# hruffieux/atlasqtl

Measured on NVIDIA B200. Metric: SNPxtrait CAVI updates/s, higher is better.
Workload: dtype f64

## Files before the change

### atlasqtl_b200/csrc/aq_sweep.cuh

```cuda
#pragma once
#include "aq_common.cuh"
#include "aq_mis.cuh"
#ifdef AQ_TIMING
#define AQ_T(i) do { long long t_ = clock64(); tacc[i] += t_ - tlast; tlast = t_; } while (0)
#define AQ_T0() long long tlast = clock64()
#else
#define AQ_T(i) do { } while (0)
#define AQ_T0() do { } while (0)
#endif

#ifndef AQ_S_FINISH_AT
#define AQ_S_FINISH_AT -1
#endif

namespace aq {

struct SweepParams {
    const int* order;
    const double* xtiles;
    size_t tile_stride;
    int nb;
    int ntiles;
    int k_base;
    int q;
    int q_pad;
    int ld_resid;
    int ncta;
    double* resid;
    double* gam;
    double* mu;
    const double* dtab;
    const double* wtab;
    const double* i0tab;
    const double* tau;
    const double* log_tau;
    const double* sig2_beta;
    double c;
    double log_sig2_inv;
    double* cs_gam;
    double* cs_gmu2;
    double* cs_b2;
    double* rsq;
    double* cs_z;
    double* rowpart;
    int rowpart_base;
    int p_pad;
    int mode;
    int nseg;
    int seg_len;
    int* seg_done;
    const unsigned long long* mbits;
    int mwords;
    const double* xnsq;
    const double* atab;
    const double* ltab;
    const double* gk;
    double* mis_out;
    long long* timing;
};

constexpr int kMaxCluster = 8;

template <int MT_, int NT_, bool CL_ = false, bool MIS_ = false>
struct SweepCfg {
    static constexpr bool kMis = MIS_;
    static constexpr int WS = 14;
    static constexpr int MT = MT_;
    static constexpr int NT = NT_;
    static constexpr bool kCl = CL_;
    static constexpr int kMmaWarps = WS;
    static constexpr int kT = MT * 8;
    static constexpr int kNPad = WS * NT * 8;
    static constexpr int kXS = kNPad + ((kNPad % 16 == 0) ? 8 : 0);
    static constexpr int kThreads = 16 * 32;
    static constexpr int kStages = 3;
    static constexpr bool kShortLogistic = CL_ || MIS_ || MT_ != 2;
    static constexpr int kSFin = (MT_ <= 2) ? AQ_S_FINISH_AT : -1;
    static constexpr size_t kTileDoubles = (size_t)kBlk * kXS + kTileTail;
    static constexpr int kSps = 8;
    static constexpr size_t kSpartDoubles = (size_t)WS * kT * kSps;
    static constexpr bool kChainSums = MT > 1;
    static constexpr bool kHelperSumsFollowers = kCl && kChainSums;
#ifdef AQ_AB_CHAIN_FWD
    static constexpr bool kChainForwards = kCl && kChainSums;
#else
    static constexpr bool kChainForwards = false;
#endif
    static constexpr size_t kSsumDoubles = (kChainSums && !kHelperSumsFollowers) ? 0 : (size_t)2 * kT * kSps;
    static constexpr size_t kDbufDoubles = (size_t)2 * kT * kBlk;
    static constexpr size_t kRsqDoubles = (size_t)WS * kT;
    static constexpr int kIoPer = kMis ? 4 : 2;
    static constexpr size_t kIoDoubles = (size_t)2 * kBlk * kIoPer * kT;
    static constexpr int kStgArrays = kMis ? 8 : 5;
    static constexpr size_t kStgDoubles = (size_t)kStgArrays * kBlk * kT;
    static constexpr size_t kGkDoubles = kMis ? (size_t)2 * 128 * kT : 0;
    static constexpr uint32_t kDeltaBytes = (uint32_t)(kT * kBlk * sizeof(double));
    static constexpr size_t kRedDoubles = kCl ? (size_t)2 * (kMaxCluster - 1) * kT * kSps : 0;
    static constexpr size_t kRsqAllDoubles = kCl ? (size_t)(kMaxCluster - 1) * kT : 0;
    static constexpr int kNumBars = 2 * kStages + 2 + 2 + 2 + 1 + 2 + 1 + 8;
    static constexpr size_t kSmemBytes = (kStages * kTileDoubles + kSpartDoubles + kSsumDoubles + kDbufDoubles + kRsqDoubles +
                                          kIoDoubles + kStgDoubles + kRedDoubles + kRsqAllDoubles + kGkDoubles) *
                                             sizeof(double) +
                                         24 * sizeof(uint64_t);
    static_assert(kNumBars <= 24, "barrier block");
    static_assert(kT <= 32, "one chain lane per trait");
    static_assert(!kMis || kT == 16, "the missing-response variant uses 16-trait tiles (its Gram band table is laid out for them)");
    static_assert(kXS % 16 == 8, "row stride must be 8 mod 16 doubles");
    static_assert(kSmemBytes <= 232448, "shared memory budget (227 KB)");
};

__device__ __forceinline__ int sp_off(int r, int t) { return r * 8 + ((((t >> 1) ^ (r >> 1)) & 3) << 1) + (t & 1); }
template <int kT>
__device__ __forceinline__ int d_off(int r, int t) { return (t >> 1) * 2 * kT + ((2 * r + (t & 1)) ^ (((t >> 1) & 1) << 3)); }

template <int N>
__device__ __forceinline__ void group_sums(double (&v)[N], int lane, int top_bit) {
    if constexpr (N > 1) {
        const bool up = (lane & top_bit) != 0;
        double w[N / 2];
#pragma unroll
        for (int i = 0; i < N / 2; ++i) {
            const double send = up ? v[i] : v[i + N / 2];
            const double keep = up ? v[i + N / 2] : v[i];
            w[i] = keep + __shfl_xor_sync(0xffffffffu, send, top_bit);
        }
        group_sums<N / 2>(w, lane, top_bit >> 1);
        v[0] = w[0];
    } else {
        v[0] += __shfl_xor_sync(0xffffffffu, v[0], 2);
        v[0] += __shfl_xor_sync(0xffffffffu, v[0], 1);
    }
}

template <class Cfg>
__device__ __forceinline__ void sum_own_partials(double (&s)[kBlk], const double* spart, uint64_t* sdone, uint64_t* sfree,
                                                 long gb, int lane, int tsum) {
    constexpr int WS = Cfg::WS, kT = Cfg::kT;
    static_assert(WS == 14, "MMA warp i sits on SMSP i % 3 for i < 12, warps 12 and 13 on SMSP 3");
    constexpr int kH = (kT <= 16) ? 2 : 1;
    const int half = (kH == 2) ? (lane >> 4) : 0;
    const uint32_t par = (uint32_t)((gb >> 1) & 1);
#pragma unroll
    for (int t = 0; t < kBlk; ++t) s[t] = 0.0;
    auto add = [&](int w) {
#pragma unroll
        for (int t = 0; t < kBlk; t += 2) {
            const double2 v = *reinterpret_cast<const double2*>(spart + w * kT * Cfg::kSps + sp_off(tsum, t));
            s[t] += v.x;
            s[t + 1] += v.y;
        }
    };
    mbar_wait(&sdone[(gb & 1) * 4 + 3], par);
    if (kH == 2) add(12 + half);
    else { add(12); add(13); }
#pragma unroll
    for (int g4 = 0; g4 < 3; ++g4) {
        mbar_wait(&sdone[(gb & 1) * 4 + g4], par);
        if (kH == 2) { add(g4 + 6 * half); add(g4 + 6 * half + 3); }
        else { add(g4); add(g4 + 3); add(g4 + 6); add(g4 + 9); }
    }
    __syncwarp();
    if (lane == 0) mbar_arrive(&sfree[0]);
}

template <class Cfg>
__device__ __forceinline__ void sum_follower_tiles(double (&s)[kBlk], const double* red, uint64_t* sred, long gb, int ncta,
                                                   int lane, int tsum) {
    constexpr int kT = Cfg::kT;
    constexpr int kH = (kT <= 16) ? 2 : 1;
    const int half = (kH == 2) ? (lane >> 4) : 0;
#pragma unroll
    for (int t = 0; t < kBlk; ++t) s[t] = 0.0;
    if (lane == 0) mbar_arrive_expect_tx(&sred[gb & 1], (uint32_t)(ncta - 1) * Cfg::kDeltaBytes);
    mbar_wait(&sred[gb & 1], (uint32_t)((gb >> 1) & 1));
    const int mid = (kH == 2) ? (ncta + 1) / 2 : ncta;
    for (int r2 = (half == 0 ? 1 : mid); r2 < (half == 0 ? mid : ncta); ++r2) {
        const double* rp = red + (size_t)((gb & 1) * (kMaxCluster - 1) + (r2 - 1)) * kT * Cfg::kSps;
#pragma unroll
        for (int t = 0; t < kBlk; t += 2) {
            const double2 v = *reinterpret_cast<const double2*>(rp + sp_off(tsum, t));
            s[t] += v.x;
            s[t + 1] += v.y;
        }
    }
    if (kH == 2) {
#pragma unroll
        for (int t = 0; t < kBlk; ++t) s[t] += __shfl_xor_sync(0xffffffffu, s[t], 16);
    }
}

template <class Cfg>
__device__ __forceinline__ void sum_s_partials(double (&s)[kBlk], const double* spart, const double* red, uint64_t* sdone,
                                               uint64_t* sfree, uint64_t* sred, long gb, int ncta, int lane, int tsum) {
    constexpr int kT = Cfg::kT;
    constexpr int kH = (kT <= 16) ? 2 : 1;
    const int half = (kH == 2) ? (lane >> 4) : 0;
    sum_own_partials<Cfg>(s, spart, sdone, sfree, gb, lane, tsum);
    if (Cfg::kCl && ncta > 1) {
        if (lane == 0) mbar_arrive_expect_tx(&sred[gb & 1], (uint32_t)(ncta - 1) * Cfg::kDeltaBytes);
        mbar_wait(&sred[gb & 1], (uint32_t)((gb >> 1) & 1));
        if (half == 0) {
            for (int r2 = 1; r2 < ncta; ++r2) {
                const double* rp = red + (size_t)((gb & 1) * (kMaxCluster - 1) + (r2 - 1)) * kT * Cfg::kSps;
#pragma unroll
                for (int t = 0; t < kBlk; t += 2) {
                    const double2 v = *reinterpret_cast<const double2*>(rp + sp_off(tsum, t));
                    s[t] += v.x;
                    s[t + 1] += v.y;
                }
            }
        }
    }
    if (kH == 2) {
#pragma unroll
        for (int t = 0; t < kBlk; ++t) s[t] += __shfl_xor_sync(0xffffffffu, s[t], 16);
    }
}

struct Unit {
    int tile, seg, b0, b1;
};
__device__ __forceinline__ Unit unit_of(const SweepParams& P, int group, int ngroups, int ju) {
    const int u = group + ju * ngroups;
    Unit w;
    w.seg = u / P.ntiles;
    w.tile = u - w.seg * P.ntiles;
    w.b0 = w.seg * P.seg_len;
    w.b1 = min(P.nb, w.b0 + P.seg_len);
    return w;
}
__device__ __forceinline__ void unit_acquire(const SweepParams& P, const Unit& w, int lane) {
    if (w.seg > 0) {
        if (lane == 0) {
            uint32_t spins = 0;
            while (ld_acquire_gpu(P.seg_done + w.tile) < w.seg) {
                __nanosleep(64);
                if (++spins == (1u << 23)) __trap();
            }
        }
        __syncwarp();
    }
}
template <class Cfg>
__device__ __forceinline__ void unit_release(const SweepParams& P, const Unit& w) {
    if (P.nseg > 1) {
        __syncwarp();
        if constexpr (Cfg::kCl) cluster_sync_all();
        else asm volatile("bar.sync 2, %0;" ::"n"(Cfg::kThreads) : "memory");
        bool leader = threadIdx.x == 0;
        if constexpr (Cfg::kCl) leader = leader && cluster_ctarank() == 0;
        if (leader) {
            __threadfence();
            st_release_gpu(P.seg_done + w.tile, w.seg + 1);
        }
    }
}

template <class Cfg>
__global__ void __launch_bounds__(Cfg::kThreads, 1) sweep_kernel(const SweepParams P) {
    constexpr int WS = Cfg::WS, MT = Cfg::MT, NT = Cfg::NT, kT = Cfg::kT, XS = Cfg::kXS;
    constexpr int kStages = Cfg::kStages;
    constexpr bool kCl = Cfg::kCl;
    constexpr bool kMis = Cfg::kMis;
    constexpr int kIoPer = Cfg::kIoPer;
    extern __shared__ __align__(128) unsigned char smem_raw[];
    double* tiles = reinterpret_cast<double*>(smem_raw);
    double* spart = tiles + kStages * Cfg::kTileDoubles;
    double* ssum = spart + Cfg::kSpartDoubles;
    double* dbuf = ssum + Cfg::kSsumDoubles;
    double* rsqs = dbuf + Cfg::kDbufDoubles;
    double* iobuf = rsqs + Cfg::kRsqDoubles;
    double* stg = iobuf + Cfg::kIoDoubles;
    double* red = stg + Cfg::kStgDoubles;
    double* rsq_all = red + Cfg::kRedDoubles;
    double* gkbuf = rsq_all + Cfg::kRsqAllDoubles;
    uint64_t* bars = reinterpret_cast<uint64_t*>(gkbuf + Cfg::kGkDoubles);
    uint64_t* full = bars;
    uint64_t* empty = bars + kStages;
    uint64_t* dready = bars + 2 * kStages;
    uint64_t* dcons = bars + 2 * kStages + 2;
    uint64_t* sred = bars + 2 * kStages + 4;
    uint64_t* rsqbar = bars + 2 * kStages + 6;
    uint64_t* inready = bars + 2 * kStages + 7;
    uint64_t* sfree = bars + 2 * kStages + 9;
    uint64_t* sdone = bars + 2 * kStages + 10;

    const int wid = threadIdx.x >> 5, lane = threadIdx.x & 31;
#ifdef AQ_TIMING
    long long tacc[16] = {0, 0, 0, 0, 0, 0, 0, 0, 0, 0, 0, 0, 0, 0, 0, 0};
#endif
    const int smsp = wid & 3, quad = wid >> 2;
    const bool is_mma = smsp != 3 || quad >= 2;
    const int mma_idx = smsp != 3 ? quad * 3 + smsp : 12 + (quad - 2);
    const bool is_chain = smsp == 3 && quad == 0;
    const bool is_helper = smsp == 3 && quad == 1;
    const bool is_producer = mma_idx == Cfg::kMmaWarps - 1 && is_mma;
    const int ncta = kCl ? P.ncta : 1;
    const int rank = kCl ? (int)cluster_ctarank() : 0;
    const int group = kCl ? (int)cluster_id_x() : (int)blockIdx.x;
    const int ngroups = kCl ? (int)cluster_count_x() : (int)gridDim.x;
    if (threadIdx.x == 0) {
        for (int s = 0; s < kStages; ++s) { mbar_init(&full[s], 1); mbar_init(&empty[s], Cfg::kMmaWarps); }
        for (int s = 0; s < 2; ++s) {
            for (int g4 = 0; g4 < 4; ++g4) mbar_init(&sdone[s * 4 + g4], g4 < 3 ? 4 : Cfg::kMmaWarps - 12);
            mbar_init(&dready[s], 1);
            mbar_init(&dcons[s], Cfg::kMmaWarps * ncta);
            mbar_init(&sred[s], 1);
            mbar_init(&inready[s], 1);
        }
        mbar_init(&rsqbar[0], ncta > 1 ? ncta - 1 : 1);
        mbar_init(&sfree[0], 1);
        fence_mbar_init();
    }
    __syncthreads();
    if (kCl) cluster_sync_all();

    const int nunits = P.ntiles * P.nseg;
    const int my_units = (nunits - group + ngroups - 1) / ngroups;
    const uint32_t tile_bytes = (uint32_t)(Cfg::kTileDoubles * sizeof(double));

    if (is_mma) {
        const int ws = mma_idx;
        const int mtid = mma_idx * 32 + lane;
        long total = 0;
        int pj = 0, pb = 0, pb1 = 0;
        if (is_producer) {
            for (int ju = 0; ju < my_units; ++ju) {
                const Unit w = unit_of(P, group, ngroups, ju);
                total += w.b1 - w.b0;
            }
            if (my_units > 0) {
                const Unit w = unit_of(P, group, ngroups, 0);
                pb = w.b0;
                pb1 = w.b1;
            }
        }
        auto load_next = [&](long it) {
            const int stage = (int)(it % kStages);
            mbar_arrive_expect_tx(&full[stage], tile_bytes);
            bulk_g2s(tiles + stage * Cfg::kTileDoubles, P.xtiles + ((size_t)pb * ncta + rank) * P.tile_stride, tile_bytes, &full[stage]);
            if (++pb == pb1 && ++pj < my_units) {
                const Unit w = unit_of(P, group, ngroups, pj);
                pb = w.b0;
                pb1 = w.b1;
            }
        };
        if (is_producer && lane == 0)
            for (long it = 0; it < kStages && it < total; ++it) load_next(it);
        const int g = lane >> 2, l = lane & 3;
        const int i0 = ws * NT * 8;
        const int ig = rank * Cfg::kNPad + i0;
        constexpr int tr0 = 0;
        const int offS = g * XS + ((i0 + 2 * l) ^ ((g & 2) << 1));
        const int offU0 = l * XS + ((i0 + g) ^ ((l & 2) << 1));
        const int offU1 = (l + 4) * XS + ((i0 + g) ^ ((l & 2) << 1));
        const int offD = d_off<kT>(tr0 + g, l);
        const int offP = sp_off(tr0 + g, 2 * l);
        uint32_t dcons_leader[2] = {0, 0}, rsqbar_leader = 0, rsq_all_leader = 0;
        if (kCl) {
            dcons_leader[0] = mapa_u32(&dcons[0], 0);
            dcons_leader[1] = mapa_u32(&dcons[1], 0);
            rsqbar_leader = mapa_u32(&rsqbar[0], 0);
            rsq_all_leader = mapa_u32(rsq_all, 0);
        }
        double acc[MT][NT][2];
        long gb = 0;
        for (int ju = 0; ju < my_units; ++ju) {
            const Unit un = unit_of(P, group, ngroups, ju);
            const int k0 = P.k_base + un.tile * kT;
            unit_acquire(P, un, lane);
#pragma unroll
            for (int mt = 0; mt < MT; ++mt)
#pragma unroll
                for (int nt = 0; nt < NT; ++nt) {
                    const double2 v = __ldcg(reinterpret_cast<const double2*>(
                        P.resid + (size_t)(k0 + tr0 + mt * 8 + g) * P.ld_resid + ig + nt * 8 + 2 * l));
                    acc[mt][nt][0] = v.x;
                    acc[mt][nt][1] = v.y;
                }
            constexpr int kSC = (MT >= 4) ? 1 : 2;
            double sa[MT][2][2];
            uint32_t mb[MT];
            if constexpr (kMis) {
#pragma unroll
                for (int mt = 0; mt < MT; ++mt) {
                    const unsigned long long* row = P.mbits + (size_t)(k0 + tr0 + mt * 8 + g) * P.mwords;
                    uint32_t bits = 0;
#pragma unroll
                    for (int nt = 0; nt < NT; ++nt)
#pragma unroll
                        for (int e = 0; e < 2; ++e) {
                            const int smp = ig + nt * 8 + 2 * l + e;
                            bits |= (uint32_t)((__ldg(row + (smp >> 6)) >> (smp & 63)) & 1ull) << (2 * nt + e);
                        }
                    mb[mt] = bits;
                }
            }
            auto s_issue = [&](long gbi) {
                const int stage = (int)(gbi % kStages);
                AQ_T0();
                mbar_wait(&full[stage], (uint32_t)((gbi / kStages) & 1));
                AQ_T(10);
                const double* xt = tiles + stage * Cfg::kTileDoubles;
#pragma unroll
                for (int mt = 0; mt < MT; ++mt) sa[mt][0][0] = sa[mt][0][1] = sa[mt][1][0] = sa[mt][1][1] = 0.0;
#pragma unroll
                for (int nt = 0; nt < NT; ++nt) {
                    const double2 xb = *reinterpret_cast<const double2*>(xt + offS + nt * 8);
#pragma unroll
                    for (int mt = 0; mt < MT; ++mt) dmma(sa[mt][0][0], sa[mt][0][1], acc[mt][nt][0], xb.x);
#pragma unroll
                    for (int mt = 0; mt < MT; ++mt) dmma(sa[mt][kSC - 1][0], sa[mt][kSC - 1][1], acc[mt][nt][1], xb.y);
                }
                AQ_T(11);
            };
            auto s_finish = [&](long gbi) {
                AQ_T0();
                if (gbi > 0) mbar_wait(&sfree[0], (uint32_t)((gbi - 1) & 1));
                AQ_T(12);
                double* sp = spart + (size_t)ws * kT * Cfg::kSps + offP;
#pragma unroll
                for (int mt = 0; mt < MT; ++mt) {
                    double2 v;
                    v.x = (kSC == 2) ? sa[mt][0][0] + sa[mt][1][0] : sa[mt][0][0];
                    v.y = (kSC == 2) ? sa[mt][0][1] + sa[mt][1][1] : sa[mt][0][1];
                    *reinterpret_cast<double2*>(sp + mt * 8 * Cfg::kSps) = v;
                }
                __syncwarp();
                if (lane == 0) mbar_arrive(&sdone[(gbi & 1) * 4 + smsp]);
                AQ_T(13);
            };
            if (P.mode == 0) {
                s_issue(gb);
                s_finish(gb);
            }
            for (int b = un.b0; b < un.b1; ++b, ++gb) {
                const bool s_next = P.mode == 0 && b + 1 < un.b1;
                if (s_next) s_issue(gb + 1);
                if (Cfg::kSFin < 0 && s_next) s_finish(gb + 1);
                const int stage = (int)(gb % kStages);
                AQ_T0();
                if (P.mode != 0) mbar_wait(&full[stage], (uint32_t)((gb / kStages) & 1));
                mbar_wait(&dready[gb & 1], (uint32_t)((gb >> 1) & 1));
                AQ_T(14);
                const double* xt = tiles + stage * Cfg::kTileDoubles;
                const double* db = dbuf + (size_t)(gb & 1) * kT * kBlk;
                if (kCl && rank == 0 && !(Cfg::kChainForwards && P.mode == 0)) {
                    constexpr int kV2 = kT * kBlk / 2;
                    const int nsend = (ncta - 1) * kV2;
                    for (int L = mtid; L < nsend; L += Cfg::kMmaWarps * 32) {
                        const int r2 = 1 + L / kV2, idx = L % kV2;
                        const double2 v = *reinterpret_cast<const double2*>(db + 2 * idx);
                        st_async_v2(mapa_u32(db + 2 * idx, r2), v.x, v.y, mapa_u32(&dready[gb & 1], r2));
                    }
                }
                double nd[MT][2];
#pragma unroll
                for (int mt = 0; mt < MT; ++mt) {
                    nd[mt][0] = db[offD + 16 * mt];
                    nd[mt][1] = db[offD + 16 * mt + 4 * kT];
                }
                if (P.mode != 0) {
                    __syncwarp();
                    if (lane == 0) {
                        if (kCl) mbar_arrive_cluster(dcons_leader[gb & 1]);
                        else mbar_arrive(&dcons[gb & 1]);
                    }
                }
#pragma unroll
                for (int nt = 0; nt < NT; nt += 2) {
                    constexpr int kLast = NT - 1;
                    const int nt1 = nt + 1 < NT ? nt + 1 : kLast;
                    const bool two = nt + 1 < NT;
                    const double x0a = xt[offU0 + nt * 8], x1a = xt[offU1 + nt * 8];
                    const double x0b = xt[offU0 + nt1 * 8], x1b = xt[offU1 + nt1 * 8];
#pragma unroll
                    for (int mt = 0; mt < MT; ++mt) dmma(acc[mt][nt][0], acc[mt][nt][1], nd[mt][0], x0a);
                    if (two) {
#pragma unroll
                        for (int mt = 0; mt < MT; ++mt) dmma(acc[mt][nt1][0], acc[mt][nt1][1], nd[mt][0], x0b);
                    }
#pragma unroll
                    for (int mt = 0; mt < MT; ++mt) dmma(acc[mt][nt][0], acc[mt][nt][1], nd[mt][1], x1a);
                    if (two) {
#pragma unroll
                        for (int mt = 0; mt < MT; ++mt) dmma(acc[mt][nt1][0], acc[mt][nt1][1], nd[mt][1], x1b);
                    }
                    if (nt == Cfg::kSFin && s_next) s_finish(gb + 1);
                }
                if (Cfg::kSFin >= NT && s_next) s_finish(gb + 1);
                if constexpr (kMis) {
#pragma unroll
                    for (int mt = 0; mt < MT; ++mt)
#pragma unroll
                        for (int nt = 0; nt < NT; ++nt) {
                            if (!((mb[mt] >> (2 * nt)) & 1u)) acc[mt][nt][0] = 0.0;
                            if (!((mb[mt] >> (2 * nt + 1)) & 1u)) acc[mt][nt][1] = 0.0;
                        }
                }
                __syncwarp();
                if (lane == 0) mbar_arrive(&empty[stage]);
                AQ_T(15);
                if (is_producer) {
                    if (lane == 0 && gb + kStages < total) {
                        mbar_wait(&empty[stage], (uint32_t)((gb / kStages) & 1));
                        load_next(gb + kStages);
                    }
                    __syncwarp();
                }
            }
#pragma unroll
            for (int mt = 0; mt < MT; ++mt) {
                double ss = 0.0;
#pragma unroll
                for (int nt = 0; nt < NT; ++nt) {
                    double2 v;
                    v.x = acc[mt][nt][0];
                    v.y = acc[mt][nt][1];
                    ss = fma(v.x, v.x, ss);
                    ss = fma(v.y, v.y, ss);
                    *reinterpret_cast<double2*>(P.resid + (size_t)(k0 + tr0 + mt * 8 + g) * P.ld_resid + ig + nt * 8 + 2 * l) = v;
                }
                ss += __shfl_xor_sync(0xffffffffu, ss, 1);
                ss += __shfl_xor_sync(0xffffffffu, ss, 2);
                if (l == 0) rsqs[ws * kT + tr0 + mt * 8 + g] = ss;
            }
            const bool last_seg = un.seg == P.nseg - 1;
            asm volatile("bar.sync 1, %0;" ::"n"(Cfg::kMmaWarps * 32) : "memory");
            if (mtid < 32 * ((kT + 31) / 32)) {
                double ss = 0.0;
                if (mtid < kT) {
#pragma unroll
                    for (int w2 = 0; w2 < WS; ++w2) ss += rsqs[w2 * kT + mtid];
                }
                if (!kCl) {
                    if (last_seg && mtid < kT && k0 + mtid < P.q) P.rsq[k0 + mtid] = ss;
                } else if (rank != 0) {
                    if (mtid < kT) st_cluster_f64(rsq_all_leader + (uint32_t)(((rank - 1) * kT + mtid) * sizeof(double)), ss);
                    __syncwarp();
                    if (mtid == 0) mbar_arrive_cluster(rsqbar_leader);
                } else {
                    if (ncta > 1) mbar_wait_cluster(&rsqbar[0], (uint32_t)(ju & 1));
                    if (mtid < kT) {
                        for (int r2 = 1; r2 < ncta; ++r2) ss += rsq_all[(r2 - 1) * kT + mtid];
                        if (last_seg && k0 + mtid < P.q) P.rsq[k0 + mtid] = ss;
                    }
                }
            }
            asm volatile("bar.sync 1, %0;" ::"n"(Cfg::kMmaWarps * 32) : "memory");
            unit_release<Cfg>(P, un);
        }
    } else if (is_chain && rank != 0) {
        constexpr int kH = (kT <= 16) ? 2 : 1;
        constexpr int kTP = kBlk / kH;
        const int half = (kH == 2) ? (lane >> 4) : 0;
        const int tl = (kH == 2) ? (lane & 15) : lane;
        const bool active = tl < kT;
        const int tls = active ? tl : 0;
        const uint32_t red_leader = mapa_u32(red, 0);
        const uint32_t sred_leader[2] = {mapa_u32(&sred[0], 0), mapa_u32(&sred[1], 0)};
        long gb = 0;
        for (int ju = 0; ju < my_units; ++ju) {
            const Unit un = unit_of(P, group, ngroups, ju);
            for (int b = un.b0; b < un.b1; ++b, ++gb) {
                if (gb >= 2) mbar_wait(&dready[gb & 1], (uint32_t)(((gb >> 1) - 1) & 1));
                if (lane == 0) mbar_arrive_expect_tx(&dready[gb & 1], Cfg::kDeltaBytes);
                if (P.mode != 0) continue;
                double s[kBlk];
                sum_own_partials<Cfg>(s, spart, sdone, sfree, gb, lane, tls);
                if (kH == 2) {
#pragma unroll
                    for (int t = 0; t < kBlk; ++t) s[t] += __shfl_xor_sync(0xffffffffu, s[t], 16);
                }
                if (active) {
                    const uint32_t dst = red_leader + (uint32_t)((((gb & 1) * (kMaxCluster - 1)) + (rank - 1)) * kT *
                                                                 Cfg::kSps * sizeof(double));
#pragma unroll
                    for (int i = 0; i < kTP; i += 2) {
                        const int t = half * kTP + i;
                        st_async_v2(dst + (uint32_t)sp_off(tl, t) * (uint32_t)sizeof(double), s[t], s[t + 1], sred_leader[gb & 1]);
                    }
                }
            }
            unit_release<Cfg>(P, un);
        }
    } else if (is_helper) {
        constexpr int kH = (kT <= 16) ? 2 : 1;
        constexpr int kTP = kBlk / kH;
        constexpr bool kStageWI = (kH == 2);
        const int half = (kH == 2) ? (lane >> 4) : 0;
        const int tl = (kH == 2) ? (lane & 15) : lane;
        const bool active = tl < kT;
        const int tls = active ? tl : 0;
        const int t0 = half * kTP;
        const bool work = P.mode == 0 && rank == 0;
        int idn[kTP], idc[kTP];
        double wn[kTP], in[kTP];
        long gb = 0;
        for (int ju = 0; ju < my_units; ++ju) {
            const Unit un = unit_of(P, group, ngroups, ju);
            if (work) {
                const int tile = un.tile;
                const int k = P.k_base + tile * kT + tls;
                const bool valid = active && k < P.q;
                double cst;
                if constexpr (kMis) cst = -(P.log_tau[k] + P.log_sig2_inv) / 2;
                else cst = -(P.log_tau[k] + P.log_sig2_inv + log(P.sig2_beta[k])) / 2;
                const double ctau = P.c * P.tau[k], inv_ctau = 1.0 / ctau;
                double sg = 0.0, sgm2 = 0.0, sb2 = 0.0, sz = 0.0;
                double ss2g = 0.0, sxgm2 = 0.0, sxs2g = 0.0, sxb2 = 0.0, sgl = 0.0;
                double xnn[kTP], s2n[kTP], lsn[kTP];
                double* rowrow = P.rowpart ? P.rowpart + (size_t)(P.rowpart_base + tile) * P.p_pad : nullptr;
                auto stage_rows = [&](int blk) {
                    constexpr int kLanesPerRow = kT / 2, kRowsPerInst = 32 / kLanesPerRow;
                    constexpr int kArrays = kMis ? 8 : (kStageWI ? 5 : 3);
                    static_assert(!kMis || kStageWI, "the missing-response variant stages all its rows");
                    const int idr = __ldg(P.order + (size_t)blk * kBlk + (lane & 7));
                    const int rsub = lane / kLanesPerRow, csub = 2 * (lane % kLanesPerRow);
                    const size_t kcol = (size_t)P.k_base + (size_t)tile * kT + csub;
#pragma unroll
                    for (int r0 = 0; r0 < kArrays * kBlk; r0 += kRowsPerInst) {
                        const int row = r0 + rsub;
                        const int a = row / kBlk, t = row % kBlk;
                        const int idt = __shfl_sync(0xffffffffu, idr, t);
                        if (row < kArrays * kBlk) {
                            const double* base = a == 0 ? P.gam : a == 1 ? P.mu : a == 2 ? P.dtab : a == 3 ? P.wtab :
                                                 a == 4 ? P.i0tab : a == 5 ? P.xnsq : a == 6 ? P.atab : P.ltab;
                            cp_async16(stg + (size_t)row * kT + csub, base + (size_t)(idt < 0 ? 0 : idt) * P.q_pad + kcol);
                        }
                    }
                    cp_async_commit();
                };
                auto stage_gk = [&](long g, int blk) {
                    if constexpr (kMis) {
                        const double* src = P.gk + (((size_t)(P.k_base / kT + tile) * P.nb + blk) * 128) * kT;
                        double* dst = gkbuf + (size_t)(g & 1) * 128 * kT;
                        for (int i = lane; i < 128 * kT / 2; i += 32) cp_async16(dst + 2 * i, src + 2 * i);
                        cp_async_commit();
                    }
                };
                auto pre = [&](long g, int blk) {
                    AQ_T0();
                    double* io = iobuf + (size_t)(g & 1) * kBlk * kIoPer * kT;
                    cp_async_wait_all();
                    __syncwarp();
#pragma unroll
                    for (int i = 0; i < kTP; ++i) {
                        const int t = t0 + i;
                        idn[i] = __ldg(P.order + (size_t)blk * kBlk + t);
                        const double go = stg[(0 * kBlk + t) * kT + tls], mo = stg[(1 * kBlk + t) * kT + tls];
                        const double dd = stg[(2 * kBlk + t) * kT + tls];
                        if (kStageWI) {
                            wn[i] = stg[(3 * kBlk + t) * kT + tls];
                            in[i] = stg[(4 * kBlk + t) * kT + tls];
                        }
                        if constexpr (kMis) {
                            const double xn = stg[(5 * kBlk + t) * kT + tls], aa = stg[(6 * kBlk + t) * kT + tls];
                            const double ls = stg[(7 * kBlk + t) * kT + tls];
                            xnn[i] = xn;
                            s2n[i] = aa * inv_ctau;
                            lsn[i] = ls;
                            if (active) {
                                io[(t * kIoPer + 0) * kT + tl] = idn[i] >= 0 ? go * mo : 0.0;
                                io[(t * kIoPer + 1) * kT + tl] = P.c * (dd - 0.5 * ls + cst);
                                io[(t * kIoPer + 2) * kT + tl] = aa;
                                io[(t * kIoPer + 3) * kT + tl] = 0.5 * P.c * aa * ctau;
                            }
                        } else if (active) {
                            io[(t * kIoPer + 0) * kT + tl] = idn[i] >= 0 ? go * mo : 0.0;
                            io[(t * kIoPer + 1) * kT + tl] = P.c * (dd + cst);
                        }
                    }
                    if (blk + 1 < un.b1) stage_rows(blk + 1);
                    if constexpr (Cfg::kHelperSumsFollowers) {
                        if (ncta > 1) {
                            double s[kBlk];
                            sum_follower_tiles<Cfg>(s, red, sred, g, ncta, lane, tls);
                            if (half == 0 && active) {
#pragma unroll
                                for (int t = 0; t < kBlk; t += 2) {
                                    double2 v;
                                    v.x = s[t];
                                    v.y = s[t + 1];
                                    *reinterpret_cast<double2*>(ssum + (size_t)(g & 1) * kT * Cfg::kSps + sp_off(tl, t)) = v;
                                }
                            }
                        }
                    }
                    if (!Cfg::kChainSums) {
                        AQ_T(4);
                        double s[kBlk];
                        sum_s_partials<Cfg>(s, spart, red, sdone, sfree, sred, g, ncta, lane, tls);
                        if (half == 0 && active) {
#pragma unroll
                            for (int t = 0; t < kBlk; t += 2) {
                                double2 v;
                                v.x = s[t];
                                v.y = s[t + 1];
                                *reinterpret_cast<double2*>(ssum + (size_t)(g & 1) * kT * Cfg::kSps + sp_off(tl, t)) = v;
                            }
                        }
                    }
                    __syncwarp();
                    if (lane == 0) mbar_arrive(&inready[g & 1]);
                    AQ_T(7);
                };
                auto post = [&](long g, int blk, const double (&ww)[kTP], const double (&ii)[kTP], const double (&xc)[kTP],
                                const double (&s2c)[kTP], const double (&lsc)[kTP]) {
                    AQ_T0();
                    mbar_wait(&dready[g & 1], (uint32_t)((g >> 1) & 1));
                    AQ_T(8);
                    if (blk + 2 < un.b1) stage_gk(g + 2, blk + 2);
                    const double* io = iobuf + (size_t)(g & 1) * kBlk * kIoPer * kT;
                    double zrow[kTP];
#pragma unroll
                    for (int i = 0; i < kTP; ++i) {
                        const int t = t0 + i;
                        const double gm = io[(t * kIoPer + 0) * kT + tls];
                        const double m = io[(t * kIoPer + 1) * kT + tls];
                        zrow[i] = 0.0;
                        if (idc[i] >= 0) {
                            const double bn = gm * m;
                            const double z = fma(gm, ww[i], ii[i]);
                            sg += gm;
                            sgm2 = fma(bn, m, sgm2);
                            sb2 = fma(bn, bn, sb2);
                            sz += z;
                            if constexpr (kMis) {
                                ss2g = fma(s2c[i], gm, ss2g);
                                sxgm2 = fma(xc[i] * bn, m, sxgm2);
                                sxs2g = fma(xc[i] * s2c[i], gm, sxs2g);
                                sxb2 = fma(xc[i] * bn, bn, sxb2);
                                sgl = fma(gm, lsc[i], sgl);
                            }
                            if (valid) {
                                const size_t off = (size_t)idc[i] * P.q_pad + k;
                                P.gam[off] = gm;
                                P.mu[off] = m;
                                if (!kCl) zrow[i] = z;
                            }
                        }
                    }
                    if (!kCl && P.rowpart) {
                        group_sums<kTP>(zrow, lane, kH == 2 ? 8 : 16);
                        const int slot = (lane >> 2) & (kTP - 1);
                        int ids = idc[0];
#pragma unroll
                        for (int i = 1; i < kTP; ++i) ids = slot == i ? idc[i] : ids;
                        if ((lane & 3) == 0 && ids >= 0) rowrow[ids] = zrow[0];
                    }
                    AQ_T(9);
                };
                stage_gk(gb, un.b0);
                if (un.b0 + 1 < un.b1) stage_gk(gb + 1, un.b0 + 1);
                stage_rows(un.b0);
                pre(gb, un.b0);
                for (int b = un.b0; b < un.b1; ++b, ++gb) {
                    double ww[kTP], ii[kTP], xc[kTP], s2c[kTP], lsc[kTP];
#pragma unroll
                    for (int i = 0; i < kTP; ++i) {
                        idc[i] = idn[i];
                        xc[i] = xnn[i];
                        s2c[i] = s2n[i];
                        lsc[i] = lsn[i];
                        if (kStageWI) {
                            ww[i] = wn[i];
                            ii[i] = in[i];
                        } else {
                            const size_t off = (size_t)(idc[i] < 0 ? 0 : idc[i]) * P.q_pad + k;
                            ww[i] = P.wtab[off];
                            ii[i] = P.i0tab[off];
                        }
                    }
                    if (b + 1 < un.b1) pre(gb + 1, b + 1);
                    post(gb, b, ww, ii, xc, s2c, lsc);
                }
                if (kH == 2) {
                    sg += __shfl_xor_sync(0xffffffffu, sg, 16);
                    sgm2 += __shfl_xor_sync(0xffffffffu, sgm2, 16);
                    sb2 += __shfl_xor_sync(0xffffffffu, sb2, 16);
                    sz += __shfl_xor_sync(0xffffffffu, sz, 16);
                    if constexpr (kMis) {
                        ss2g += __shfl_xor_sync(0xffffffffu, ss2g, 16);
                        sxgm2 += __shfl_xor_sync(0xffffffffu, sxgm2, 16);
                        sxs2g += __shfl_xor_sync(0xffffffffu, sxs2g, 16);
                        sxb2 += __shfl_xor_sync(0xffffffffu, sxb2, 16);
                        sgl += __shfl_xor_sync(0xffffffffu, sgl, 16);
                    }
                }
                unit_acquire(P, un, lane);
                if constexpr (kMis) {
                    if (valid && half == 0) {
                        double* o = P.mis_out + k;
                        o[(size_t)kMisGam * P.q_pad] = sg;
                        o[(size_t)kMisGamMu2 * P.q_pad] = sgm2;
                        o[(size_t)kMisS2Gam * P.q_pad] = ss2g;
                        o[(size_t)kMisXnGamMu2 * P.q_pad] = sxgm2;
                        o[(size_t)kMisXnS2Gam * P.q_pad] = sxs2g;
                        o[(size_t)kMisXnBeta2 * P.q_pad] = sxb2;
                        o[(size_t)kMisZ * P.q_pad] = sz;
                        o[(size_t)kMisGamLogS2 * P.q_pad] = sgl;
                    }
                } else if (valid && half == 0) {
                    if (un.seg > 0) {
                        sg += __ldcg(P.cs_gam + k);
                        sgm2 += __ldcg(P.cs_gmu2 + k);
                        sb2 += __ldcg(P.cs_b2 + k);
                        sz += __ldcg(P.cs_z + k);
                    }
                    P.cs_gam[k] = sg;
                    P.cs_gmu2[k] = sgm2;
                    P.cs_b2[k] = sb2;
                    P.cs_z[k] = sz;
                }
            }
            unit_release<Cfg>(P, un);
        }
    } else if (is_chain) {
        const int tl = lane;
        const bool active = tl < kT;
        const int tls = active ? tl : 0;
        const int tsum0 = (kT <= 16) ? (lane & 15) : lane;
        const int tsum = tsum0 < kT ? tsum0 : 0;
        auto publish = [&](long gb, const double (&nd)[kBlk]) {
            double* dblk = dbuf + (size_t)(gb & 1) * kT * kBlk;
            if constexpr (Cfg::kChainForwards) {
                if (P.mode == 0 && active) {
                    for (int r2 = 1; r2 < ncta; ++r2) {
                        const uint32_t rbar = mapa_u32(&dready[gb & 1], r2);
#pragma unroll
                        for (int t = 0; t < kBlk; t += 2)
                            st_async_v2(mapa_u32(dblk + d_off<kT>(tl, t), r2), nd[t], nd[t + 1], rbar);
                    }
                }
            }
            if (active) {
#pragma unroll
                for (int t = 0; t < kBlk; t += 2) {
                    double2 v;
                    v.x = nd[t];
                    v.y = nd[t + 1];
                    *reinterpret_cast<double2*>(dblk + d_off<kT>(tl, t)) = v;
                }
            }
            __syncwarp();
            if (lane == 0) mbar_arrive(&dready[gb & 1]);
        };
        long gb = 0;
        for (int ju = 0; ju < my_units; ++ju) {
            const Unit un = unit_of(P, group, ngroups, ju);
            const int k = P.k_base + un.tile * kT + tls;
            const bool valid = active && k < P.q;
            if (P.mode == 0) {
                double a = 0.0, bq = 0.0;
                if constexpr (!kMis) {
                    const double sig2 = P.sig2_beta[k];
                    a = P.c * sig2 * P.tau[k];
                    bq = P.c * a * a / (2.0 * sig2);
                }
                double corr[kBlk];
#pragma unroll
                for (int t = 0; t < kBlk; ++t) corr[t] = 0.0;
                for (int b = un.b0; b < un.b1; ++b, ++gb) {
                    AQ_T0();
                    const int stage = (int)(gb % kStages);
                    mbar_wait(&full[stage], (uint32_t)((gb / kStages) & 1));
                    const double* gband = kMis ? gkbuf + (size_t)(gb & 1) * 128 * kT + tsum
                                               : tiles + stage * Cfg::kTileDoubles + kBlk * XS;
                    constexpr int gstride = kMis ? kT : 1;
                    double* io = iobuf + (size_t)(gb & 1) * kBlk * kIoPer * kT;
                    double s[kBlk], bo[kBlk], ap[kBlk], nd[kBlk], av[kMis ? kBlk : 1], bv[kMis ? kBlk : 1];
                    if constexpr (Cfg::kHelperSumsFollowers) {
                        AQ_T(0);
                        sum_own_partials<Cfg>(s, spart, sdone, sfree, gb, lane, tsum);
                        if (kT <= 16) {
#pragma unroll
                            for (int t = 0; t < kBlk; ++t) s[t] += __shfl_xor_sync(0xffffffffu, s[t], 16);
                        }
                    }
                    mbar_wait(&inready[gb & 1], (uint32_t)((gb >> 1) & 1));
#pragma unroll
                    for (int t = 0; t < kBlk; ++t) {
                        bo[t] = io[(t * kIoPer + 0) * kT + tsum];
                        ap[t] = io[(t * kIoPer + 1) * kT + tsum];
                        if constexpr (kMis) {
                            av[t] = io[(t * kIoPer + 2) * kT + tsum];
                            bv[t] = io[(t * kIoPer + 3) * kT + tsum];
                        }
                    }
                    if constexpr (Cfg::kHelperSumsFollowers) {
                        if (ncta > 1) {
                            const double* sp0 = ssum + (size_t)(gb & 1) * kT * Cfg::kSps;
#pragma unroll
                            for (int t = 0; t < kBlk; t += 2) {
                                const double2 v = *reinterpret_cast<const double2*>(sp0 + sp_off(tsum, t));
                                s[t] += v.x;
                                s[t + 1] += v.y;
                            }
                        }
                    } else if (Cfg::kChainSums) {
                        AQ_T(0);
                        sum_s_partials<Cfg>(s, spart, red, sdone, sfree, sred, gb, ncta, lane, tsum);
                    } else {
                        AQ_T(0);
                        const double* sp0 = ssum + (size_t)(gb & 1) * kT * Cfg::kSps;
#pragma unroll
                        for (int t = 0; t < kBlk; t += 2) {
                            const double2 v = *reinterpret_cast<const double2*>(sp0 + sp_off(tsum, t));
                            s[t] = v.x;
                            s[t + 1] = v.y;
                        }
                    }
#pragma unroll
                    for (int t = 0; t < kBlk; ++t) {
                        s[t] = fma(bo[t], gband[(t * 16 + 8 + t) * gstride], s[t] + corr[t]);
                        corr[t] = 0.0;
                    }
                    AQ_T(1);
#pragma unroll
                    for (int t = 0; t < kBlk; ++t) {
                        const double st = s[t];
                        const double m = (kMis ? av[kMis ? t : 0] : a) * st;
                        const double x = fma(st * st, -(kMis ? bv[kMis ? t : 0] : bq), ap[t]);
                        const double gm = logistic_neg<Cfg::kShortLogistic>(x);
                        const double dlt = fma(gm, m, -bo[t]);
                        const double* grow = gband + t * 16 * gstride;
#pragma unroll
                        for (int u = t + 1; u < kBlk; ++u) s[u] = fma(-grow[(8 + u) * gstride], dlt, s[u]);
#pragma unroll
                        for (int u = 0; u < kBlk; ++u) corr[u] = fma(-grow[u * gstride], dlt, corr[u]);
                        nd[t] = -dlt;
                        if (active) {
                            io[(t * kIoPer + 0) * kT + tl] = gm;
                            io[(t * kIoPer + 1) * kT + tl] = m;
                        }
                    }
                    AQ_T(2);
                    publish(gb, nd);
                    AQ_T(3);
                }
            } else {
                double sg = 0.0, sgm2 = 0.0, sb2 = 0.0, sxg = 0.0, sxgm2 = 0.0, sxb2 = 0.0;
                for (int b = un.b0; b < un.b1; ++b, ++gb) {
                    const int stage = (int)(gb % kStages);
                    mbar_wait(&full[stage], (uint32_t)((gb / kStages) & 1));
                    const int* ids = reinterpret_cast<const int*>(tiles + stage * Cfg::kTileDoubles + kBlk * XS + 128);
                    double nd[kBlk];
#pragma unroll
                    for (int t = 0; t < kBlk; ++t) {
                        const int idt = ids[t];
                        const size_t off = (size_t)(idt < 0 ? 0 : idt) * P.q_pad + k;
                        const double go = P.gam[off], mo = P.mu[off];
                        const double bo = idt >= 0 ? go * mo : 0.0;
                        if (idt >= 0) {
                            sg += go;
                            sgm2 = fma(bo, mo, sgm2);
                            sb2 = fma(bo, bo, sb2);
                            if constexpr (kMis) {
                                const double xn = P.xnsq[off];
                                sxg = fma(xn, go, sxg);
                                sxgm2 = fma(xn * bo, mo, sxgm2);
                                sxb2 = fma(xn * bo, bo, sxb2);
                            }
                        }
                        nd[t] = -bo;
                    }
                    if (gb >= 2) {
                        if (kCl) mbar_wait_cluster(&dcons[gb & 1], (uint32_t)(((gb >> 1) - 1) & 1));
                        else mbar_wait(&dcons[gb & 1], (uint32_t)(((gb >> 1) - 1) & 1));
                    }
                    publish(gb, nd);
                }
                unit_acquire(P, un, lane);
                if constexpr (kMis) {
                    if (valid) {
                        double* o = P.mis_out + k;
                        o[(size_t)kMisGam * P.q_pad] = sg;
                        o[(size_t)kMisGamMu2 * P.q_pad] = sgm2;
                        o[(size_t)kMisS2Gam * P.q_pad] = sb2;
                        o[(size_t)kMisXnGamMu2 * P.q_pad] = sxgm2;
                        o[(size_t)kMisXnS2Gam * P.q_pad] = sxg;
                        o[(size_t)kMisXnBeta2 * P.q_pad] = sxb2;
                    }
                } else if (valid) {
                    if (un.seg > 0) {
                        sg += __ldcg(P.cs_gam + k);
                        sgm2 += __ldcg(P.cs_gmu2 + k);
                        sb2 += __ldcg(P.cs_b2 + k);
                    }
                    P.cs_gam[k] = sg;
                    P.cs_gmu2[k] = sgm2;
                    P.cs_b2[k] = sb2;
                }
            }
            unit_release<Cfg>(P, un);
        }
    }
#ifdef AQ_TIMING
    if (blockIdx.x == 0 && lane == 0 && P.timing && (is_chain || is_helper || wid == 0))
        for (int i = 0; i < 16; ++i)
            if (tacc[i]) atomicAdd(reinterpret_cast<unsigned long long*>(P.timing) + i, (unsigned long long)tacc[i]);
#endif
    if (kCl) {
        __syncwarp();
        cluster_sync_all();
    }
}

}
```

Before: 6.403 billion.

## Split MMA warps into two trait groups with double-buffered S partials

For the non-cluster, non-missing MT=2 configuration, the 14 MMA warps are reorganised into two trait groups. Each warp owns one 8-trait M tile over twice as many N columns, so there are 7 warp slices instead of 14. The S-partial buffer is double-buffered by block parity, which removes the sfree wait and arrive handshake. The sum stage also reads fewer partial slices. The change trades more N work per warp and four independent accumulation chains against less per-warp reduction and synchronisation, and it adds timing instrumentation for barrier waits.

```diff
diff --git a/atlasqtl_b200/csrc/aq_sweep.cuh b/atlasqtl_b200/csrc/aq_sweep.cuh
--- a/atlasqtl_b200/csrc/aq_sweep.cuh
+++ b/atlasqtl_b200/csrc/aq_sweep.cuh
@@ -72,13 +72,19 @@
     static constexpr int kT = MT * 8;
     static constexpr int kNPad = WS * NT * 8;
     static constexpr int kXS = kNPad + ((kNPad % 16 == 0) ? 8 : 0);
+    static constexpr int kTG = (MT_ == 2 && !CL_ && !MIS_) ? 2 : 1;
+    static constexpr int kSL = WS / kTG;
+    static constexpr int kMW = MT / kTG;
+    static constexpr int kNW = NT * kTG;
     static constexpr int kThreads = 16 * 32;
     static constexpr int kStages = 3;
     static constexpr bool kShortLogistic = CL_ || MIS_ || MT_ != 2;
     static constexpr int kSFin = (MT_ <= 2) ? AQ_S_FINISH_AT : -1;
     static constexpr size_t kTileDoubles = (size_t)kBlk * kXS + kTileTail;
     static constexpr int kSps = 8;
-    static constexpr size_t kSpartDoubles = (size_t)WS * kT * kSps;
+    static constexpr int kSBufs = kTG;
+    static constexpr size_t kSpartOne = (size_t)kSL * kT * kSps;
+    static constexpr size_t kSpartDoubles = kSBufs * kSpartOne;
     static constexpr bool kChainSums = MT > 1;
     static constexpr bool kHelperSumsFollowers = kCl && kChainSums;
 #ifdef AQ_AB_CHAIN_FWD
@@ -106,6 +112,7 @@
     static_assert(kT <= 32, "one chain lane per trait");
     static_assert(!kMis || kT == 16, "the missing-response variant uses 16-trait tiles (its Gram band table is laid out for them)");
     static_assert(kXS % 16 == 8, "row stride must be 8 mod 16 doubles");
+    static_assert(kTG == 1 || (kTG == 2 && MT == 2 && kT == 16), "two trait groups: one 8-trait M tile per warp, half-warp sums");
     static_assert(kSmemBytes <= 232448, "shared memory budget (227 KB)");
 };
 
@@ -134,33 +141,47 @@
 
 template <class Cfg>
 __device__ __forceinline__ void sum_own_partials(double (&s)[kBlk], const double* spart, uint64_t* sdone, uint64_t* sfree,
-                                                 long gb, int lane, int tsum) {
+                                                 long gb, int lane, int tsum, long long* twait = nullptr) {
     constexpr int WS = Cfg::WS, kT = Cfg::kT;
     static_assert(WS == 14, "MMA warp i sits on SMSP i % 3 for i < 12, warps 12 and 13 on SMSP 3");
     constexpr int kH = (kT <= 16) ? 2 : 1;
     const int half = (kH == 2) ? (lane >> 4) : 0;
     const uint32_t par = (uint32_t)((gb >> 1) & 1);
+    const double* sp = spart + (Cfg::kSBufs == 2 ? (size_t)(gb & 1) * Cfg::kSpartOne : 0);
 #pragma unroll
     for (int t = 0; t < kBlk; ++t) s[t] = 0.0;
     auto add = [&](int w) {
 #pragma unroll
         for (int t = 0; t < kBlk; t += 2) {
-            const double2 v = *reinterpret_cast<const double2*>(spart + w * kT * Cfg::kSps + sp_off(tsum, t));
+            const double2 v = *reinterpret_cast<const double2*>(sp + w * kT * Cfg::kSps + sp_off(tsum, t));
             s[t] += v.x;
             s[t + 1] += v.y;
         }
     };
-    mbar_wait(&sdone[(gb & 1) * 4 + 3], par);
-    if (kH == 2) add(12 + half);
+    auto wait = [&](int g4) {
+#ifdef AQ_TIMING
+        const long long t_ = clock64();
+        mbar_wait(&sdone[(gb & 1) * 4 + g4], par);
+        if (twait) *twait += clock64() - t_;
+#else
+        mbar_wait(&sdone[(gb & 1) * 4 + g4], par);
+#endif
+    };
+    wait(3);
+    if (Cfg::kTG == 2) { if (half) add(6); }
+    else if (kH == 2) add(12 + half);
     else { add(12); add(13); }
 #pragma unroll
     for (int g4 = 0; g4 < 3; ++g4) {
-        mbar_wait(&sdone[(gb & 1) * 4 + g4], par);
-        if (kH == 2) { add(g4 + 6 * half); add(g4 + 6 * half + 3); }
+        wait(g4);
+        if (Cfg::kTG == 2) add(2 * g4 + half);
+        else if (kH == 2) { add(g4 + 6 * half); add(g4 + 6 * half + 3); }
         else { add(g4); add(g4 + 3); add(g4 + 6); add(g4 + 9); }
     }
-    __syncwarp();
-    if (lane == 0) mbar_arrive(&sfree[0]);
+    if (Cfg::kSBufs == 1) {
+        __syncwarp();
+        if (lane == 0) mbar_arrive(&sfree[0]);
+    }
 }
 
 template <class Cfg>
@@ -191,11 +212,12 @@
 
 template <class Cfg>
 __device__ __forceinline__ void sum_s_partials(double (&s)[kBlk], const double* spart, const double* red, uint64_t* sdone,
-                                               uint64_t* sfree, uint64_t* sred, long gb, int ncta, int lane, int tsum) {
+                                               uint64_t* sfree, uint64_t* sred, long gb, int ncta, int lane, int tsum,
+                                               long long* twait = nullptr) {
     constexpr int kT = Cfg::kT;
     constexpr int kH = (kT <= 16) ? 2 : 1;
     const int half = (kH == 2) ? (lane >> 4) : 0;
-    sum_own_partials<Cfg>(s, spart, sdone, sfree, gb, lane, tsum);
+    sum_own_partials<Cfg>(s, spart, sdone, sfree, gb, lane, tsum, twait);
     if (Cfg::kCl && ncta > 1) {
         if (lane == 0) mbar_arrive_expect_tx(&sred[gb & 1], (uint32_t)(ncta - 1) * Cfg::kDeltaBytes);
         mbar_wait(&sred[gb & 1], (uint32_t)((gb >> 1) & 1));
@@ -320,7 +342,9 @@
     const uint32_t tile_bytes = (uint32_t)(Cfg::kTileDoubles * sizeof(double));
 
     if (is_mma) {
-        const int ws = mma_idx;
+        constexpr int kMW = Cfg::kMW, kNW = Cfg::kNW, kSL = Cfg::kSL;
+        const int tg = Cfg::kTG == 2 ? (quad & 1) : 0;
+        const int ws = Cfg::kTG == 2 ? (smsp < 3 ? 2 * smsp + (quad >> 1) : 6) : mma_idx;
         const int mtid = mma_idx * 32 + lane;
         long total = 0;
         int pj = 0, pb = 0, pb1 = 0;
@@ -348,9 +372,9 @@
         if (is_producer && lane == 0)
             for (long it = 0; it < kStages && it < total; ++it) load_next(it);
         const int g = lane >> 2, l = lane & 3;
-        const int i0 = ws * NT * 8;
+        const int i0 = ws * kNW * 8;
         const int ig = rank * Cfg::kNPad + i0;
-        constexpr int tr0 = 0;
+        const int tr0 = tg * kMW * 8;
         const int offS = g * XS + ((i0 + 2 * l) ^ ((g & 2) << 1));
         const int offU0 = l * XS + ((i0 + g) ^ ((l & 2) << 1));
         const int offU1 = (l + 4) * XS + ((i0 + g) ^ ((l & 2) << 1));
@@ -363,24 +387,24 @@
             rsqbar_leader = mapa_u32(&rsqbar[0], 0);
             rsq_all_leader = mapa_u32(rsq_all, 0);
         }
-        double acc[MT][NT][2];
+        double acc[kMW][kNW][2];
         long gb = 0;
         for (int ju = 0; ju < my_units; ++ju) {
             const Unit un = unit_of(P, group, ngroups, ju);
             const int k0 = P.k_base + un.tile * kT;
             unit_acquire(P, un, lane);
 #pragma unroll
-            for (int mt = 0; mt < MT; ++mt)
-#pragma unroll
-                for (int nt = 0; nt < NT; ++nt) {
+            for (int mt = 0; mt < kMW; ++mt)
+#pragma unroll
+                for (int nt = 0; nt < kNW; ++nt) {
                     const double2 v = __ldcg(reinterpret_cast<const double2*>(
                         P.resid + (size_t)(k0 + tr0 + mt * 8 + g) * P.ld_resid + ig + nt * 8 + 2 * l));
                     acc[mt][nt][0] = v.x;
                     acc[mt][nt][1] = v.y;
                 }
-            constexpr int kSC = (MT >= 4) ? 1 : 2;
-            double sa[MT][2][2];
-            uint32_t mb[MT];
+            constexpr int kSC = (kMW >= 4) ? 1 : (Cfg::kTG == 2 ? 4 : 2);
+            double sa[kMW][kSC][2];
+            uint32_t mb[kMW];
             if constexpr (kMis) {
 #pragma unroll
                 for (int mt = 0; mt < MT; ++mt) {
@@ -403,27 +427,35 @@
                 AQ_T(10);
                 const double* xt = tiles + stage * Cfg::kTileDoubles;
 #pragma unroll
-                for (int mt = 0; mt < MT; ++mt) sa[mt][0][0] = sa[mt][0][1] = sa[mt][1][0] = sa[mt][1][1] = 0.0;
-#pragma unroll
-                for (int nt = 0; nt < NT; ++nt) {
+                for (int mt = 0; mt < kMW; ++mt)
+#pragma unroll
+                    for (int c = 0; c < kSC; ++c) sa[mt][c][0] = sa[mt][c][1] = 0.0;
+#pragma unroll
+                for (int nt = 0; nt < kNW; ++nt) {
                     const double2 xb = *reinterpret_cast<const double2*>(xt + offS + nt * 8);
-#pragma unroll
-                    for (int mt = 0; mt < MT; ++mt) dmma(sa[mt][0][0], sa[mt][0][1], acc[mt][nt][0], xb.x);
-#pragma unroll
-                    for (int mt = 0; mt < MT; ++mt) dmma(sa[mt][kSC - 1][0], sa[mt][kSC - 1][1], acc[mt][nt][1], xb.y);
+                    const int ca = (kSC == 4) ? (2 * nt) & 3 : 0, cb = (kSC == 4) ? (2 * nt + 1) & 3 : kSC - 1;
+#pragma unroll
+                    for (int mt = 0; mt < kMW; ++mt) dmma(sa[mt][ca][0], sa[mt][ca][1], acc[mt][nt][0], xb.x);
+#pragma unroll
+                    for (int mt = 0; mt < kMW; ++mt) dmma(sa[mt][cb][0], sa[mt][cb][1], acc[mt][nt][1], xb.y);
                 }
                 AQ_T(11);
             };
             auto s_finish = [&](long gbi) {
                 AQ_T0();
-                if (gbi > 0) mbar_wait(&sfree[0], (uint32_t)((gbi - 1) & 1));
+                if (Cfg::kSBufs == 1 && gbi > 0) mbar_wait(&sfree[0], (uint32_t)((gbi - 1) & 1));
                 AQ_T(12);
-                double* sp = spart + (size_t)ws * kT * Cfg::kSps + offP;
-#pragma unroll
-                for (int mt = 0; mt < MT; ++mt) {
+                double* sp = spart + (Cfg::kSBufs == 2 ? (size_t)(gbi & 1) * Cfg::kSpartOne : 0) + (size_t)ws * kT * Cfg::kSps + offP;
+                auto chains = [&](int mt, int e) {
+                    if constexpr (kSC == 4) return (sa[mt][0][e] + sa[mt][1][e]) + (sa[mt][2][e] + sa[mt][3][e]);
+                    else if constexpr (kSC == 2) return sa[mt][0][e] + sa[mt][1][e];
+                    else return sa[mt][0][e];
+                };
+#pragma unroll
+                for (int mt = 0; mt < kMW; ++mt) {
                     double2 v;
-                    v.x = (kSC == 2) ? sa[mt][0][0] + sa[mt][1][0] : sa[mt][0][0];
-                    v.y = (kSC == 2) ? sa[mt][0][1] + sa[mt][1][1] : sa[mt][0][1];
+                    v.x = chains(mt, 0);
+                    v.y = chains(mt, 1);
                     *reinterpret_cast<double2*>(sp + mt * 8 * Cfg::kSps) = v;
                 }
                 __syncwarp();
@@ -454,9 +486,9 @@
                         st_async_v2(mapa_u32(db + 2 * idx, r2), v.x, v.y, mapa_u32(&dready[gb & 1], r2));
                     }
                 }
-                double nd[MT][2];
-#pragma unroll
-                for (int mt = 0; mt < MT; ++mt) {
+                double nd[kMW][2];
+#pragma unroll
+                for (int mt = 0; mt < kMW; ++mt) {
                     nd[mt][0] = db[offD + 16 * mt];
                     nd[mt][1] = db[offD + 16 * mt + 4 * kT];
                 }
@@ -468,32 +500,32 @@
                     }
                 }
 #pragma unroll
-                for (int nt = 0; nt < NT; nt += 2) {
-                    constexpr int kLast = NT - 1;
-                    const int nt1 = nt + 1 < NT ? nt + 1 : kLast;
-                    const bool two = nt + 1 < NT;
+                for (int nt = 0; nt < kNW; nt += 2) {
+                    constexpr int kLast = kNW - 1;
+                    const int nt1 = nt + 1 < kNW ? nt + 1 : kLast;
+                    const bool two = nt + 1 < kNW;
                     const double x0a = xt[offU0 + nt * 8], x1a = xt[offU1 + nt * 8];
                     const double x0b = xt[offU0 + nt1 * 8], x1b = xt[offU1 + nt1 * 8];
 #pragma unroll
-                    for (int mt = 0; mt < MT; ++mt) dmma(acc[mt][nt][0], acc[mt][nt][1], nd[mt][0], x0a);
+                    for (int mt = 0; mt < kMW; ++mt) dmma(acc[mt][nt][0], acc[mt][nt][1], nd[mt][0], x0a);
                     if (two) {
 #pragma unroll
-                        for (int mt = 0; mt < MT; ++mt) dmma(acc[mt][nt1][0], acc[mt][nt1][1], nd[mt][0], x0b);
-                    }
-#pragma unroll
-                    for (int mt = 0; mt < MT; ++mt) dmma(acc[mt][nt][0], acc[mt][nt][1], nd[mt][1], x1a);
+                        for (int mt = 0; mt < kMW; ++mt) dmma(acc[mt][nt1][0], acc[mt][nt1][1], nd[mt][0], x0b);
+                    }
+#pragma unroll
+                    for (int mt = 0; mt < kMW; ++mt) dmma(acc[mt][nt][0], acc[mt][nt][1], nd[mt][1], x1a);
                     if (two) {
 #pragma unroll
-                        for (int mt = 0; mt < MT; ++mt) dmma(acc[mt][nt1][0], acc[mt][nt1][1], nd[mt][1], x1b);
+                        for (int mt = 0; mt < kMW; ++mt) dmma(acc[mt][nt1][0], acc[mt][nt1][1], nd[mt][1], x1b);
                     }
                     if (nt == Cfg::kSFin && s_next) s_finish(gb + 1);
                 }
-                if (Cfg::kSFin >= NT && s_next) s_finish(gb + 1);
+                if (Cfg::kSFin >= kNW && s_next) s_finish(gb + 1);
                 if constexpr (kMis) {
 #pragma unroll
-                    for (int mt = 0; mt < MT; ++mt)
-#pragma unroll
-                        for (int nt = 0; nt < NT; ++nt) {
+                    for (int mt = 0; mt < kMW; ++mt)
+#pragma unroll
+                        for (int nt = 0; nt < kNW; ++nt) {
                             if (!((mb[mt] >> (2 * nt)) & 1u)) acc[mt][nt][0] = 0.0;
                             if (!((mb[mt] >> (2 * nt + 1)) & 1u)) acc[mt][nt][1] = 0.0;
                         }
@@ -510,10 +542,10 @@
                 }
             }
 #pragma unroll
-            for (int mt = 0; mt < MT; ++mt) {
+            for (int mt = 0; mt < kMW; ++mt) {
                 double ss = 0.0;
 #pragma unroll
-                for (int nt = 0; nt < NT; ++nt) {
+                for (int nt = 0; nt < kNW; ++nt) {
                     double2 v;
                     v.x = acc[mt][nt][0];
                     v.y = acc[mt][nt][1];
@@ -531,7 +563,7 @@
                 double ss = 0.0;
                 if (mtid < kT) {
 #pragma unroll
-                    for (int w2 = 0; w2 < WS; ++w2) ss += rsqs[w2 * kT + mtid];
+                    for (int w2 = 0; w2 < kSL; ++w2) ss += rsqs[w2 * kT + mtid];
                 }
                 if (!kCl) {
                     if (last_seg && mtid < kT && k0 + mtid < P.q) P.rsq[k0 + mtid] = ss;
@@ -900,7 +932,11 @@
                         }
                     } else if (Cfg::kChainSums) {
                         AQ_T(0);
+#ifdef AQ_TIMING
+                        sum_s_partials<Cfg>(s, spart, red, sdone, sfree, sred, gb, ncta, lane, tsum, &tacc[5]);
+#else
                         sum_s_partials<Cfg>(s, spart, red, sdone, sfree, sred, gb, ncta, lane, tsum);
+#endif
                     } else {
                         AQ_T(0);
                         const double* sp0 = ssum + (size_t)(gb & 1) * kT * Cfg::kSps;
```

After: 6.478 billion (median of 6 runs). +1.2%, better.
